# yavuzmurattas/Infrared-Colorization-with-ResNet-Generator-and-PatchGAN

Hardware: AMD Instinct MI355X
Metric: GAN train-step img/s (G+D fwd/bwd) at 256×256, 1/2/4/8 MI355X (higher is better)
Workload: dtype bf16; 1 GPU; GAN train step 256x256, batch 16/GPU, bf16 (BASELINE configs[1]); global_batch=16, img_size=256, height=256, width=256, parallelism=dp1

## Files before the change

### include/irgan.h

```cpp
#ifndef IRGAN_H
#define IRGAN_H
#include <stdint.h>
#include <stddef.h>

#if defined(__GNUC__) || defined(__clang__)
#define IRGAN_API __attribute__((visibility("default")))
#else
#define IRGAN_API
#endif

#ifdef __cplusplus
extern "C" {
#endif

typedef void* irgan_stream_t;

IRGAN_API int irgan_build_id(char* buf, int32_t len);

enum { IRGAN_F32 = 0, IRGAN_BF16 = 1, IRGAN_FP8 = 2 };
enum { IRGAN_PAD_ZERO = 0, IRGAN_PAD_REFLECT = 1 };
enum { IRGAN_ACT_NONE = 0, IRGAN_ACT_RELU = 1, IRGAN_ACT_LRELU = 2, IRGAN_ACT_TANH = 3 };
enum { IRGAN_OK = 0, IRGAN_EINVAL = 1001, IRGAN_EUNSUPPORTED = 1002 };

typedef struct irgan_conv_desc {
    int32_t N, H, W, Cin, ldx, xoff;
    int32_t Ho, Wo, Cout, ldy, yoff;
    int32_t OH, OW, omy, ooy, omx, oox;
    int32_t KH, KW, sy, sx, c0y, c0x;
    int32_t pad_mode;
    int32_t act;
    int32_t accumulate;
    int32_t dtype;
    int32_t out_dtype;
    int32_t mask_act;
    int32_t ldm, moff;
    int32_t cin_real;
    int32_t flags;
} irgan_conv_desc;
enum { IRGAN_CONV_DETERMINISTIC = 1 };

IRGAN_API int irgan_conv_fwd(const irgan_conv_desc* d, const void* x, const void* w,
                   const float* bias, void* y, const void* mask, irgan_stream_t s);

IRGAN_API int irgan_conv_fwd_stats(const irgan_conv_desc* d, const void* x, const void* w,
                         const float* bias, void* y, void* part, int32_t* nb, irgan_stream_t s);

IRGAN_API int irgan_conv_fwd_fp8(const irgan_conv_desc* d, const void* x, const void* w, const float* dqx,
                       const float* dqw, const float* bias, void* y, void* part, int32_t* nb,
                       irgan_stream_t s);

IRGAN_API int irgan_conv_wgrad_fp8(const irgan_conv_desc* d, const void* x8, const void* dy8, const float* dqx,
                         const float* dqdy, float* dw, float* ws, int64_t ws_floats, irgan_stream_t s);

enum { IRGAN_FP8_AMAX_PARTS = 256 };

IRGAN_API int irgan_fp8_quant(const void* x, int32_t dt, int64_t P, int32_t C, int32_t ldx, int32_t xoff,
                    void* y, int32_t ldy, int32_t yoff, const float* q, uint32_t* amax,
                    irgan_stream_t s);
IRGAN_API int irgan_fp8_scale(uint32_t* amax, int32_t n, float* q, float* dq, int32_t reset, irgan_stream_t s);
typedef struct irgan_fp8_job {
    const void* src;
    void* dst;
    int64_t n;
    int32_t slot, reserved;
} irgan_fp8_job;
IRGAN_API int irgan_fp8_quant_batch(const void* jobs, int32_t njobs, int64_t max_n, const float* q,
                          uint32_t* amax, irgan_stream_t s);

// ... 276 lines not shown
```

### infrared-colorization-with-resnet-generator-and-patchgan_amd/csrc/conv_pp.hip

```cpp
#include "conv_pp_kernel.h"

namespace irgan_res64 {
bool ok(const irgan_conv_desc* d);
int launch(const irgan_conv_desc* d, const void* x, const void* w, const float* bias, void* y, const void* mask,
           float2* part, hipStream_t st, void* ypool = nullptr);
}

namespace {

constexpr bool use_one(int) { return true; }
constexpr bool split128(int) { return true; }

#ifndef PP_BN_MODEL
#define PP_BN_MODEL 1
#endif
int narrow_bn(const irgan_conv_desc* d) {
    const long patches = (long)d->N * irgan_cdiv(d->Ho, PH) * irgan_cdiv(d->Wo, PW);
    if (patches * (d->Cout / 256) >= 160) {
        if (PP_BN_MODEL) {
            const long cus = irgan_cu_count();
            const long r256 = irgan_cdiv(patches * (d->Cout / 256), cus);
            const long r128 = irgan_cdiv(patches * (d->Cout / 128), cus);
            if (r128 * 0.575 <= 0.9 * r256) return 128;
        }
// ... 196 lines not shown
#define PPS(KHV, BNV, ONEV, ...)                                                                                   \
    conv_pp_kernel<KHV, KHV, BNV, false, true, false, ONEV, ##__VA_ARGS__><<<blocks, 512, 0, st>>>(                  \
        *d, (const bf16_t*)x, (const bf16_t*)w, bias, y, nullptr, ntn, tpx, tpy, swz, (float2*)part)
    const bool one = bn == 64 && use_one(d->Cin);
    if (s2d) {
        if (bn == 256) PPS(2, 256, false, true);
        else if (bn == 128) PPS(2, 128, false, true);
        else PPS(2, 64, true, true);
    } else if (k33) {
        if (bn == 256) PPS(3, 256, false);
        else if (bn == 128) PPS(3, 128, false);
        else { if (one) PPS(3, 64, true); else PPS(3, 64, false); }
    } else {
        if (bn == 256) PPS(4, 256, false);
        else if (bn == 128) PPS(4, 128, false);
        else { if (one) PPS(4, 64, true); else PPS(4, 64, false); }
    }
#undef PPS
    IRGAN_LAUNCH_CHECK();
    *nb = tpx * tpy;
    return 0;
}

extern "C" int irgan_conv_fwd_pool(const irgan_conv_desc* d, const void* x, const void* w, const float* bias, void* y,
                                   void* yp, irgan_stream_t s) {
    if (!d || !x || !w || !yp) return IRGAN_EINVAL;
    if ((long)d->N * d->Ho * d->Wo <= 0) return 0;
    if (!irgan_res64::ok(d) || d->accumulate || d->mask_act || d->Ho % 2 || d->Wo % 2 || d->Ho != d->OH ||
        d->Wo != d->OW || d->omy != 1 || d->omx != 1 || d->ooy || d->oox ||
        (long)d->N * (d->Ho / 2) * (d->Wo / 2) * d->Cout * 2 >= (1L << 31))
        return IRGAN_EUNSUPPORTED;
    irgan_res64::launch(d, x, w, bias, y, nullptr, nullptr, (hipStream_t)s, yp);
    IRGAN_LAUNCH_CHECK();
    return 0;
}

extern "C" int irgan_conv_fwd_fp8(const irgan_conv_desc* d, const void* x, const void* w, const float* dqx,
                                  const float* dqw, const float* bias, void* y, void* part, int32_t* nb,
                                  irgan_stream_t s) {
    if (!d || !x || !w || !dqx || !dqw || !y || (part && !nb)) return IRGAN_EINVAL;
    if ((long)d->N * d->Ho * d->Wo <= 0 || d->Cout <= 0) return 0;
    const bool k33 = d->KH == 3 && d->KW == 3;
    if (d->dtype != IRGAN_FP8 || d->out_dtype != IRGAN_BF16 || d->act == IRGAN_ACT_TANH || d->sy != 1 || d->sx != 1 ||
        d->Cin % 128 || !k33 || d->Cout % 64 || d->Cout == 192 || d->ldx % 16 || d->xoff % 16 || d->mask_act ||
        (long)d->N * d->H * d->W * d->ldx >= (1L << 30) || (long)d->Cout * 9 * d->Cin >= (1L << 30))
        return IRGAN_EUNSUPPORTED;
// ... 26 lines not shown
```

### infrared-colorization-with-resnet-generator-and-patchgan_amd/csrc/conv_pp_kernel.h

```cpp

#pragma once
#include <type_traits>

#include "conv_epilogue.h"

#ifndef PP_EXP
#define PP_EXP 0
#endif
#define PPX(b) ((PP_EXP & (b)) != 0)

namespace {

IRGAN_HD int lds_off(int row, int chunk) { return row * 128 + ((chunk ^ (row & 7)) << 4); }

IRGAN_HD void sched_fence() { __builtin_amdgcn_sched_barrier(0); }
IRGAN_HD void phase_barrier() {
    sched_fence();
#if !PPX(8)
    lds_barrier();
#endif
    sched_fence();
}
IRGAN_HD void wait_lgkm0() { asm volatile("s_waitcnt lgkmcnt(0)" ::: "memory"); }

constexpr int PH = 16, PW = 16;
constexpr int HPMAX = 46;
constexpr int HBYTES = HPMAX * 1024;
// ... 29 lines not shown
    };
    if (row) {
        const int line = y == 1 ? 0 : 1;
        add(line, x + 1);
        if (x == 1) { add(line, 0); add(2, y + 1); }
        if (x == W - 2) { add(line, W + 1); add(3, y + 1); }
    } else {
        add(x == 1 ? 2 : 3, y + 1);
    }
}
IRGAN_HD void ring_line_apply(const float (&v)[8], uint4& o) {
    const uint32_t wd[4] = {o.x, o.y, o.z, o.w};
    uint32_t o4[4];
#pragma unroll
    for (int k = 0; k < 4; ++k)
        o4[k] = pk_bf16(__uint_as_float(wd[k] << 16) + v[2 * k], __uint_as_float(wd[k] & 0xffff0000u) + v[2 * k + 1]);
    o = make_uint4(o4[0], o4[1], o4[2], o4[3]);
}

struct PhaseTab {
    const bf16_t* w[4];
    int c0y[4], c0x[4], ooy[4], oox[4];
};
IRGAN_HD int pick4(const int (&a)[4], int i) { return i == 0 ? a[0] : (i == 1 ? a[1] : (i == 2 ? a[2] : a[3])); }

template <int KH, int KW, int BN, bool ACC, bool STATS = false, bool F8 = false, bool ONE = false, bool S2D = false,
          bool PH4 = false>
__global__ __launch_bounds__(512, ONE ? 2 : 1) void conv_pp_kernel(const irgan_conv_desc d, const bf16_t* __restrict__ x,
                                                         const bf16_t* __restrict__ w, const float* __restrict__ bias,
                                                         void* __restrict__ y, const void* __restrict__ mask,
                                                         int ntn, int tpx, int tpy, int swz,
                                                         float2* __restrict__ part = nullptr,
                                                         const float* __restrict__ dqx = nullptr,
                                                         const float* __restrict__ dqw = nullptr,
                                                         const float* __restrict__ rg = nullptr,
                                                         const PhaseTab tab = PhaseTab{}) {
    constexpr int ESZ = F8 ? 1 : 2, CHN = 128 / ESZ;
    const char* const xb = (const char*)x;
    const char* wb = (const char*)w;
    constexpr int TAPS = KH * KW, HWd = PW + KW - 1, HROWS = (PH + KH - 1) * HWd, HP = (HROWS + 7) / 8;
    constexpr int BBYTES = PP<BN>::BBYTES, NJ = PP<BN>::NJ, WU = PP<BN>::WU, RSB = PP<BN>::RSB;
    constexpr int LDS = ONE ? HBYTES + 2 * BBYTES : PP<BN>::LDS;
    static_assert(!ONE || (BN == 64 && 256 * RSB <= LDS && !F8), "single-halo variant: staging must fit");
    constexpr int MI = PP<BN>::MIW, RW = PP<BN>::RW;
    constexpr int HS = 2;
    constexpr int NP = F8 ? MI / 2 : 1, NQ = F8 ? NJ / 2 : 1;
    static_assert(!F8 || (MI % 2 == 0 && NJ % 2 == 0), "fp8: 32 x 32 fragments");
    static_assert(HP <= HPMAX && HP > 32 && TAPS >= 2, "halo pieces per wave are 4 to 6");
    static_assert(!S2D || (KH == 2 && KW == 2 && !F8), "space-to-depth: the 2x2 form of a 4x4 stride-2 conv");
    static_assert(!PH4 || (!S2D && !F8 && !STATS), "four-phase backward-data: plain bf16");
    __shared__ __attribute__((aligned(1024))) char smem[LDS];
    char* const sH = smem;
    char* const sB = smem + (ONE ? 1 : 2) * HBYTES;

    const int tid = threadIdx.x, lane = tid & 63;
    const int wid = __builtin_amdgcn_readfirstlane(tid >> 6);
    const int grp = wid >> 2, wn = wid & 3;
    const int prow = grp * 8 + (wn % RW) * MI;
    const int cb = (wn / RW) * NJ * 16;
    int t = xcd_tile(blockIdx.x, gridDim.x, swz);
    const int nt = t % ntn;
    t /= ntn;
    int c0y = d.c0y, c0x = d.c0x, ooy = d.ooy, oox = d.oox;
    if constexpr (PH4) {
        const int ph = t & 3;
        t >>= 2;
        c0y = pick4(tab.c0y, ph);
        c0x = pick4(tab.c0x, ph);
        ooy = pick4(tab.ooy, ph);
        oox = pick4(tab.oox, ph);
        wb = (const char*)(ph == 0 ? tab.w[0] : (ph == 1 ? tab.w[1] : (ph == 2 ? tab.w[2] : tab.w[3])));
    }
    const int pxi = t % tpx;
    t /= tpx;
// ... 28 lines not shown
    const uint32_t wbytes = (uint32_t)((long)d.Cout * Kw * ESZ);
    const uint32_t b_off = (uint32_t)((n0 + wid * WU * 8 + sub) * Kw * ESZ + chunk * 16);
    auto issue_halo = [&](int c) {
        char* dst = sH + (ONE ? 0 : (c & 1) * HBYTES);
        const int cc = S2D ? c % cpp : c, ph = S2D ? c / cpp : 0;
        const i32x4 rs = make_rsrc(xb + cc * 128, xbytes - cc * 128);
        int lsub = sub;
        asm volatile("" : "+v"(lsub));
#pragma unroll
        for (int u = 0; u < 6; ++u)
            if (u < nh) blds16(rs, halo_off(u, lsub, ph), dst + (u * 8 + wid) * 1024);
    };
    auto issue_w = [&](int c, int tp, int stage) {
        int kcol = tp * d.Cin + c * CHN;
        if constexpr (S2D) {
            const int ph = c / cpp;
            kcol = ((2 * (tp >> 1) + (ph >> 1)) * 4 + 2 * (tp & 1) + (ph & 1)) * d.Cin + (c % cpp) * CHN;
        }
        const i32x4 rs = make_rsrc(wb + kcol * ESZ, wbytes - kcol * ESZ);
        char* dst = sB + stage * BBYTES + wid * WU * 1024;
#pragma unroll
        for (int u = 0; u < WU; ++u) blds16(rs, b_off, (uint32_t)(u * 8 * Kw * ESZ), dst + u * 1024);
    };
    auto reload_halo = [&](int c) {
        issue_halo(c);
        wait_vmcnt<0>();
        phase_barrier();
    };
    auto retire = [&](bool halo_now) {
        if (!halo_now) wait_vmcnt<0>();
        else if (nh == 6) wait_vmcnt<6>();
        else if (nh == 5) wait_vmcnt<5>();
        else wait_vmcnt<4>();
    };

    f32x4 acc[F8 ? 1 : MI][F8 ? 1 : NJ];
    f32x16 acc32[NP][NQ];
    if constexpr (F8) {
#pragma unroll
        for (int p = 0; p < NP; ++p)
#pragma unroll
            for (int q = 0; q < NQ; ++q)
#pragma unroll
                for (int r = 0; r < 16; ++r) acc32[p][q][r] = 0.f;
    } else {
#pragma unroll
        for (int i = 0; i < MI; ++i)
#pragma unroll
            for (int j = 0; j < NJ; ++j) acc[i][j] = f32x4{0.f, 0.f, 0.f, 0.f};
    }
    uint4 af[F8 ? 1 : MI], bfr[F8 ? 1 : NJ];
    v8i_t pf8[NP], wf8[NQ];
    issue_w(0, 0, 0);
    issue_halo(0);
    issue_w(0, 1, 1);
    wait_vmcnt<WU>();
    phase_barrier();
    if (grp == 1) phase_barrier();

    const int arow0 = (prow + (F8 ? (lane >> 4) & 1 : 0)) * HWd + (lane & 15);
    const int brow0 = cb + (lane & (F8 ? 31 : 15));
    const int g0 = F8 ? lane >> 5 : lane >> 4;
    const int bb0 = lds_off(brow0, g0), bb1 = lds_off(brow0, 4 + g0);
    int tsw[8];
#pragma unroll
    for (int k8 = 0; k8 < 8; ++k8) tsw[k8] = (g0 ^ ((arow0 + k8) & 7)) << 4;
#pragma unroll 1
    for (int c = 0; c < nchunk; ++c) {
        const int hb = arow0 * 128 + (ONE ? 0 : (c & 1) * HBYTES);
        const bool more = c + 1 < nchunk;
#pragma unroll
        for (int tp = 0; tp < TAPS; ++tp) {
            const int ty = tp / KW, tx = tp % KW;
            const int k = c * TAPS + tp;
            const char* B = sB + (k & 1) * BBYTES;
            const bool last_k = !more && tp == TAPS - 1;
            const bool halo_now = tp == 0 && more && !ONE;
            const bool reload = ONE && more && tp == TAPS - 1;
#pragma unroll
            for (int h = 0; h < HS; ++h) {
                const int bb = h ? bb1 : bb0;
                int hbp = hb;
                asm volatile("" : "+v"(hbp));
                if constexpr (F8) {
#pragma unroll
                    for (int q = 0; q < NQ; ++q)
                        wf8[q] = cat8(*(const i32x4*)(B + bb + q * 4096), *(const i32x4*)(B + (bb ^ 32) + q * 4096));
#pragma unroll
                    for (int p = 0; p < NP; ++p) {
                        const int K = (2 * p + ty) * HWd + tx;
                        const int sw = tsw[K & 7] ^ (h * 64);
                        pf8[p] = cat8(*(const i32x4*)(sH + (hbp + sw) + K * 128),
                                      *(const i32x4*)(sH + (hbp + (sw ^ 32)) + K * 128));
                    }
                } else {
#if !PPX(4)
#pragma unroll
                for (int j = 0; j < NJ; ++j) bfr[j] = *(const uint4*)(B + bb + j * 2048);
#pragma unroll
                for (int i = 0; i < MI; ++i) {
                    const int K = (i + ty) * HWd + tx;
                    af[i] = *(const uint4*)(sH + (hbp + (tsw[K & 7] ^ (h * 64))) + K * 128);
                }
#else
                if (k == 0 && h == 0) {
#pragma unroll
// ... 336 lines not shown
```

### infrared-colorization-with-resnet-generator-and-patchgan_amd/csrc/norm_rows.h

```cpp
#pragma once
#include "common.h"

#include <algorithm>
#include <initializer_list>

namespace {

constexpr int TPB = 256;
constexpr int V = 8;
constexpr int FC = 8, FS = 32;

struct Slice {
    const void* p;
    int dt, ld, off;
};
struct OSlice {
    void* p;
    int dt, ld, off;
};


inline bool dt_ok(int dt) { return dt == IRGAN_F32 || dt == IRGAN_BF16; }
inline bool act_ok(int act) { return act >= IRGAN_ACT_NONE && act <= IRGAN_ACT_LRELU; }
inline bool slice_ok(int C, int ld, int off) { return off >= 0 && (long)off + C <= ld; }
// ... 60 lines not shown
            u.z = pk_bf16(v[4], v[5]);
            u.w = pk_bf16(v[6], v[7]);
            *(uint4*)((bf16_t*)p + i) = u;
        } else {
            *(float4*)((float*)p + i) = make_float4(v[0], v[1], v[2], v[3]);
            *(float4*)((float*)p + i + 4) = make_float4(v[4], v[5], v[6], v[7]);
        }
    } else {
        stv(p, dt, i, v[0]);
    }
}

IRGAN_HD float act_fwd(float h, int act) {
    if (act == IRGAN_ACT_RELU) return h > 0.f ? h : 0.f;
    if (act == IRGAN_ACT_LRELU) return h > 0.f ? h : 0.2f * h;
    return h;
}
IRGAN_HD float act_grad(float h, int act) {
    if (act == IRGAN_ACT_RELU) return h > 0.f ? 1.f : 0.f;
    if (act == IRGAN_ACT_LRELU) return h > 0.f ? 1.f : 0.2f;
    return 1.f;
}

struct Lay {
    int CL, RP, cl, rl;
    __device__ Lay(int C, int VW) {
        CL = (C + VW - 1) / VW;
        if (CL > TPB) CL = TPB;
        RP = TPB / CL;
        cl = threadIdx.x % CL;
        rl = threadIdx.x / CL;
    }
    __device__ Lay(int CL_, int RP_, int cl_, int rl_) : CL(CL_), RP(RP_), cl(cl_), rl(rl_) {}
};

enum RowOrder { ROWS_TREE, ROWS_CHAINS };
IRGAN_HD bool rows_tree_ok(int CL) { return CL <= 64 && (64 % CL) == 0; }
IRGAN_HD RowOrder in_row_order(int CL) { return rows_tree_ok(CL) ? ROWS_TREE : ROWS_CHAINS; }

template <typename T, int VW, typename Emit>
IRGAN_HD void block_reduce(T* a0, T* a1, const Lay& L, RowOrder order, bool on, int cb, int c, int C, T* s0, T* s1,
                           Emit emit) {
    if (order == ROWS_TREE) {
        for (int o = L.CL; o < 64; o <<= 1) {
#pragma unroll
            for (int k = 0; k < VW; ++k) {
// ... 67 lines not shown
```

### infrared-colorization-with-resnet-generator-and-patchgan_amd/engine.py

```python
from __future__ import annotations

import math
import os
from collections import OrderedDict
from contextlib import nullcontext as _nullcontext
from typing import NamedTuple

import torch

from . import ops
from .ops import (ACT_LRELU, ACT_NONE, ACT_RELU, ACT_TANH, BF16, F32, PAD_REFLECT, PAD_ZERO, ConvSpec, Feat,
                  PackedConv)

IMAGENET_MEAN = (0.485, 0.456, 0.406)
IMAGENET_STD = (0.229, 0.224, 0.225)



def g_param_shapes(input_nc=1, output_nc=3, ngf=64, n_blocks=9, no_antialias=False, no_antialias_up=False,
                   use_bias=True, padding_type="reflect", use_dropout=False, batch_norm=False):
    s = OrderedDict()
    use_bias = use_bias and not batch_norm

    def conv(key, shape, normed=True):
# ... 287 lines not shown
    @staticmethod
    def _red(bufs: Buffers, N, C):
        return bufs.flat("in_red", 2 * N * C)

    @staticmethod
    def _no_fp8():
        raise NotImplementedError("the fp8 path runs with InstanceNorm (norm='instance')")

    def fwd(self, bufs: Buffers, name: str, x: Feat, y: Feat, act, res: Feat = None, xhat=None, nb=0, q8=None):
        mr = self._stats(bufs, name, x, nb)
        ops.in_apply(x, mr, y, act=act, res=res, xhat=xhat, q8=q8 and q8.side)
        if q8 is not None:
            q8.finish(y)

    def _stats(self, bufs: Buffers, name: str, x: Feat, nb):
        work = self._work(bufs, x.N, x.C)
        mr = bufs.get("mr_" + name, (x.N * x.C * 2,), torch.float32)
        if nb:
            ops.in_finalize(x, work, nb, mr)
        else:
            ops.in_stats(x, work, mr)
        return mr

    def _conv(self, bufs: Buffers, pc, x: Feat, z: Feat, conv8=None):
        work = self._work(bufs, z.N, z.C)
        if conv8 is not None:
            w8, dqw, x8, dqx = conv8
            return ops.conv_fwd_fp8(pc, w8, dqw, x8, dqx, z, part=work)
        nb = ops.conv_fwd_stats(pc, x, z, work) if INLayer.fused_stats else 0
        if not nb:
            ops.conv_fwd(pc, x, z)
        return nb

    def conv_fwd(self, bufs: Buffers, name: str, pc, x: Feat, z: Feat, y: Feat, act, res: Feat = None, conv8=None,
                 q8=None):
        self.fwd(bufs, name, z, y, act, res=res, nb=self._conv(bufs, pc, x, z, conv8), q8=q8)

    def conv_stats(self, bufs: Buffers, name: str, pc, x: Feat, z: Feat, conv8=None):
        return self._stats(bufs, name, z, self._conv(bufs, pc, x, z, conv8))

    def resample_fwd(self, bufs: Buffers, name: str, pc, x: Feat, z: Feat, a_name: str, act, y: Feat, fused, plain,
                     conv8=None, q8=None):
        mr = self.conv_stats(bufs, name, pc, x, z, conv8=conv8)
        side = q8.side if q8 is not None else None
        taken = INLayer.fused_resample and (fused(z, mr, act, y, q8=side) if side is not None else
                                            fused(z, mr, act, y))
        if not taken:
            a = Feat(bufs.get(a_name, (z.N, z.H, z.W, z.C), z.t.dtype))
            ops.in_apply(z, mr, a, act=act)
            plain(a, y)
        if q8 is not None:
            q8.finish(y, taken)

    def bwd(self, bufs: Buffers, name: str, dy: Feat, z: Feat, act, dx: Feat, db=None, dy2: Feat = None, q8=None,
            wgrad=True):
        N, C = z.N, z.C
        work = self._work(bufs, N, C)
        red = self._red(bufs, N, C)
        mr = bufs.d["mr_" + name]
        ops.in_backward(dy, z, act, mr, work, red, dx, db=db if INLayer.sum_bias_grad else None, dy2=dy2,
                        q8=q8.side if q8 is not None and not INLayer.sum_bias_grad else None)
        if q8 is not None:
# ... 221 lines not shown
        A = self.eng.f8a
        if st.calib and self.s_calib is not None:
            return st.x1_8c, A.dqp(self.s_calib)
        return st.x8[self.name], ops.Pi(st.dq_used, self.rec.s_x) if used else A.dqp(self.rec.s_x)

    def _conv8(self, st):
        return (*self._w8(self.rec.w_fwd), *self._x8(st)) if st.on[self.group] else None

    def feed(self, st, x: Feat):
        if st.on[self.group]:
            self.eng.f8a.quant(self.rec.s_x, x, st.x8[self.name], record=not st.frozen)

    def side(self, st, sl=None):
        if not st.on[self.group] or (st.calib and self.group == "ud"):
            return None
        x8 = st.x8[self.name]
        return ops.Fp8Out(self.eng.f8a, self.rec.s_x, x8.sl(*sl) if sl else x8, record=not st.frozen)

    def calibrate(self, st, x: Feat):
        if st.calib and self.group == "ud":
            slot, x8 = (self.s_calib, st.x1_8c) if self.s_calib is not None else (self.rec.s_x, st.x8[self.name])
            self.eng.f8a.calibrate(slot, x, x8)

    def fwd(self, g: Buffers, st, x: Feat, z: Feat, y: Feat, act, res: Feat = None, nxt: "GenConv" = None):
        if self.xp:
            xp = Feat(g.get(self.xp, (x.N, x.H + 2, x.W + 2, x.C), self.eng.tdt))
            ops.pad(x, xp, 1, "replicate")
            x = xp
        self.norm.conv_fwd(g, self.name, self.pc, x, z, y, act, res=res, conv8=self._conv8(st),
                           q8=nxt.side(st) if nxt else None)

    def resample_fwd(self, g: Buffers, st, x: Feat, z: Feat, a_name, act, y: Feat, fused, plain):
        self.norm.resample_fwd(g, self.name, self.pc, x, z, a_name, act, y, fused, plain, conv8=self._conv8(st))

    def bwd(self, g: Buffers, st, dy: Feat, z: Feat, act, dz: Feat, x: Feat, dx: Feat, accumulate=False, padbuf=None,
            pend: list = None, resample=None):
        e, on = self.eng, st.on[self.group]
        dz8 = Feat(g.get(self.dy8, (*dz.t.shape[:3], dz.C), torch.float8_e4m3fn)) if on else None
        db, q8 = e._bgrad(self.key + ".bias"), ops.Fp8Out(e.f8a, self.rec.s_dy, dz8) if on else None
        if resample is not None:
            self.norm.resample_bwd(g, self.name, dy, z, act, dz, *resample, db=db, q8=q8)
        else:
            self.norm.bwd(g, self.name, dy, z, act, dz, db=db, q8=q8)
        if on:
            self._wgrad(st, x, dz, dz8)
            if self.s_calib is not None:
                st.x1_8c = None
            ops.conv_dgrad_fp8(self.pc, *self._w8(self.rec.w_flip), dz8, e.f8a.dqp(self.rec.s_dy), dz, dx,
                               accumulate=accumulate)
            return
        if self.group != "res":
            self._wgrad(st, x, dz)
        if self.xp:
# ... 188 lines not shown
        self.norms["inc"].conv_fwd(g, "inc", self.inc, ir_t, z0, x0, ACT_RELU)
        if self.no_aa:
            z1 = Feat(g.get("z1", (B, H1, W1, c1), T))
            ops.conv_fwd(self.down1, x0, z1)
            self.norms["down1"].fwd(g, "down1", z1, x1, ACT_RELU)
        else:
            z1 = Feat(g.get("z1", (B, H, W, c1), T))
            self.norms["down1"].resample_fwd(g, "down1", self.down1, x0, z1, "a1", ACT_RELU, x1, ops.blur_down_in,
                                             ops.blur_down, q8=D2.side(st))
            D2.calibrate(st, x1)
        h = Feat(g.get("h0", (B, H2, W2, c2), T))
        if self.no_aa:
            z2 = Feat(g.get("z2", (B, H2, W2, c2), T))
            ops.conv_fwd(self.down2, x1, z2)
            self.norms["down2"].fwd(g, "down2", z2, h, ACT_RELU)
        else:
            z2 = Feat(g.get("z2", (B, H1, W1, c2), T))
            D2.resample_fwd(g, st, x1, z2, "a2", ACT_RELU, h, ops.blur_down_in, ops.blur_down)
        if self.blocks:
            self.blocks[0][0].feed(st, h)
        for b, (ra, rb) in enumerate(self.blocks):
            r1 = Feat(g.get(f"r1_{b}", (B, H2, W2, c2), T))
            t = None if t8_only else Feat(g.get(f"t{b}", (B, H2, W2, c2), T))
            ra.fwd(g, st, h, r1, t, ACT_RELU, nxt=rb)
            if self.use_dropout and train:
                t, t1 = Feat(g.get(f"td{b}", (B, H2, W2, c2), T)), t
                ops.dropout(t1, t, g.state["dropout_seed"] + 2 * b)
            r2 = Feat(g.get(f"r2_{b}", (B, H2, W2, c2), T))
            hn = Feat(g.get(f"h{b + 1}", (B, H2, W2, c2), T))
            rb.fwd(g, st, t, r2, hn, ACT_NONE, res=h, nxt=self.blocks[b + 1][0] if b + 1 < self.n_blocks else None)
            h = hn
        self._fp8_roll(st, "res", "fwd", snapshot=True)
        y1 = Feat(cat1, 0, c2)
        if self.no_aa_up:
            self._convt(self.up1_up, h, y1, g, "ut1")
        else:
            q8 = U1.side(st, (0, c2))
            ops.upsample(h, y1, q8=q8 and q8.side)
        U1.calibrate(st, Feat(cat1))
        z3 = Feat(g.get("z3", (B, H1, W1, c1), T))
        y2 = Feat(cat2, 0, c1)
        if self.no_aa_up:
            a3 = Feat(g.get("a3", (B, H1, W1, c1), T))
            U1.fwd(g, st, Feat(cat1), z3, a3, ACT_RELU)
            self._convt(self.up2_up, a3, y2, g, "ut2")
        else:
            U1.resample_fwd(g, st, Feat(cat1), z3, "a3", ACT_RELU, y2, ops.upsample_in, ops.upsample)
        self._fp8_roll(st, "ud", "cat", snapshot=True)
        z4 = Feat(g.get("z4", (B, H, W, c0), T))
        a4 = Feat(g.get("a4", (B, H, W, c0), T))
        self.norms["up2"].conv_fwd(g, "up2", self.up2, Feat(cat2), z4, a4, ACT_RELU)
        fake = g.get("fake", (B, H, W, self.output_nc), torch.float32)
        ops.conv_fwd(self.outc, a4, Feat(fake), act=ACT_TANH)
# ... 132 lines not shown
        self.packs = [_pc(store, k, ConvSpec(chans[i], chans[i + 1], 4, s, 1, PAD_ZERO), dtype)
                      for i, (k, s, _) in enumerate(self.LAYERS)]
        self.norms = [make_norm(norm, store, f"model.{int(k.split('.')[1]) + 1}") if n else None
                      for (k, _, n) in self.LAYERS]
        self.norm_type, self.training = norm, True
        self.bn_sync = None
        self.bufs = Buffers(store.device)

    def pack(self):
        if self._pack_batch is None:
            self._pack_batch = ops.PackBatch(self.packs)
        self._pack_batch.run()

    def forward(self, din: Feat, tag="", bufs: Buffers = None, groups: int = 1, bn_sync: bool = False) -> torch.Tensor:
        g, T = bufs or self.bufs, self.tdt
        if self.norm_type == "batch":
            for nrm in self.norms:
                if nrm is not None:
                    nrm.configure(training=self.training, groups=groups, repeat=1,
                                  sync=self.bn_sync if bn_sync else None)
        x = din
        acts, pre = [din], {}
        g.state[tag] = (acts, pre)
        for i, pc in enumerate(self.packs):
            Ho, Wo = pc.spec.out_hw(x.H, x.W)
            last = i == len(self.packs) - 1
            y = Feat(g.get(f"{tag}e{i}", (x.N, Ho, Wo, pc.spec.cout), torch.float32 if last else T))
            if i == 0:
                ops.conv_fwd(pc, x, y, act=ACT_LRELU)
            elif last:
                if not ops.patch_head_fwd(pc, x, y.t):
                    ops.conv_fwd(pc, x, y)
            else:
                z = Feat(g.get(f"{tag}z{i}", (x.N, Ho, Wo, pc.spec.cout), T))
                self.norms[i].conv_fwd(g, f"{tag}n{i}", pc, x, z, y, ACT_LRELU)
                pre[i] = z
            acts.append(y)
            x = y
        return x.t

    def backward(self, dout: torch.Tensor, want_wgrad=True, want_dinput=False, tag="", bufs: Buffers = None,
                 ready=None):
        g, T, S = bufs or self.bufs, self.tdt, self.store
        acts, pre = g.state[tag]
        G = S.grad
        n = len(self.packs)
        def logits_grad():
            dbuf = g.zeros(f"{tag}dout_t", tuple(dout.shape[:3]) + (8,), T)
            ops.axpby(Feat(dout), 1.0, Feat(dbuf, 0, dout.shape[3]))
            return Feat(dbuf, 0, self.packs[-1].cout_eff)
        dy = None
        for i in reversed(range(n)):
            pc, key = self.packs[i], self.LAYERS[i][0]
            x = acts[i]
            if dy is None and not (i == n - 1 and ops.is_patch_head(pc, x)):
                dy = logits_grad()
            bias_sum = None
            if i == n - 1:
# ... 438 lines not shown
```

### infrared-colorization-with-resnet-generator-and-patchgan_amd/ops.py

```python
from __future__ import annotations

import ctypes
import math
import os

import torch

from . import _lib
from ._lib import (ACT_LRELU, ACT_NONE, ACT_RELU, ACT_TANH, BF16, F32, FP8, IN_PARTS, PAD_REFLECT,
                   PAD_ZERO)

TORCH_DT = {F32: torch.float32, BF16: torch.bfloat16, FP8: torch.float8_e4m3fn}


def dt_code(t: torch.Tensor) -> int:
    if t.dtype == torch.float32:
        return F32
    if t.dtype == torch.bfloat16:
        return BF16
    if t.dtype == torch.float8_e4m3fn:
        return FP8
    raise TypeError(f"unsupported dtype {t.dtype}")


# ... 289 lines not shown
    Ho, Wo = s.out_hw(x.H, x.W)
    if pc.dtype != BF16 or yp.dt != BF16 or yp.off or yp.ld != s.cout or Ho % 2 or Wo % 2:
        return False
    assert (yp.N, yp.H, yp.W, yp.C) == (x.N, Ho // 2, Wo // 2, s.cout) and x.C == pc.cin_eff
    if y is not None:
        assert (y.H, y.W, y.C, y.N, y.dt) == (Ho, Wo, s.cout, x.N, BF16)
    d = _fwd_desc(s, x, y if y is not None else yp, pc.cin_eff, pc.dtype, BF16, act, y_sized=y is not None)
    return TIMER.wrap(conv_tag("fwdpool", s, (x.H, x.W), x.N), lambda: _try(
        "irgan_conv_fwd_pool", ctypes.byref(d), x.ptr, P(pc.fwd), P(pc.bias), y.ptr if y is not None else None,
        yp.ptr, stream()))


def conv_fwd_stats(pc: PackedConv, x: Feat, y: Feat, part: torch.Tensor) -> int:
    s = pc.spec
    if pc.dtype != BF16 or y.dt != BF16 or s.cout % 64 or s.cout == 192 or (s.stride != 1 and s.k != 4):
        return 0
    assert y.C == s.cout and x.C == pc.cin_eff, "conv_fwd shape mismatch"
    d = _fwd_desc(s, x, y, pc.cin_eff, pc.dtype, y.dt, cin_real=s.cin if s.cin < pc.cin_eff else 0)
    nb = ctypes.c_int32(0)
    ran = TIMER.wrap(conv_tag("fwd", s, (x.H, x.W), x.N), lambda: _try(
        "irgan_conv_fwd_stats", ctypes.byref(d), x.ptr, P(pc.fwd), P(pc.bias), y.ptr, P(part), ctypes.byref(nb),
        stream()))
    return int(nb.value) if ran else 0


PATCH_HEAD = [os.environ.get("IRGAN_NO_PATCH_HEAD") != "1"]


def is_patch_head(pc: PackedConv, x: Feat) -> bool:
    s = pc.spec
    return (PATCH_HEAD[0] and pc.dtype == BF16 and x.dt == BF16 and s.cout == 1 and s.k == 4 and s.stride == 1
            and s.pad == 1 and s.mode == PAD_ZERO and s.cin == x.C == 512)


def patch_head_fwd(pc: PackedConv, x: Feat, y: torch.Tensor) -> bool:
    if not is_patch_head(pc, x):
        return False
    assert y.dtype == torch.float32 and tuple(y.shape) == (x.N, x.H - 1, x.W - 1, 1) and y.is_contiguous()

    ws = _wgrad_ws(y.device)

    return TIMER.wrap(conv_tag("fwd", pc.spec, (x.H, x.W), x.N), lambda: _try(
        "irgan_patch_head_fwd", x.ptr, x.N, x.H, x.W, x.C, x.ld, x.off, P(pc.fwd),
        P(pc.bias) if pc.bias is not None else None, P(y), P(ws), ws.numel(), stream()))


# ... 893 lines not shown
```

Before: 1323 img/s.

## Fuse instance-norm apply and activation into next conv's halo load

```diff
diff --git a/include/irgan.h b/include/irgan.h
--- a/include/irgan.h
+++ b/include/irgan.h
@@ -44,6 +44,14 @@
 
 IRGAN_API int irgan_conv_fwd_stats(const irgan_conv_desc* d, const void* x, const void* w,
                          const float* bias, void* y, void* part, int32_t* nb, irgan_stream_t s);
+
+IRGAN_API int irgan_conv_fwd_norm_in(const irgan_conv_desc* d, const void* z_in, const float* mr, int32_t act_in,
+                           const void* res, const void* xhat, const void* t8, void* t_out, int32_t ldt,
+                           int32_t toff, const void* w, const float* bias, void* y, irgan_stream_t s);
+IRGAN_API int irgan_conv_fwd_norm_in_stats(const irgan_conv_desc* d, const void* z_in, const float* mr,
+                                 int32_t act_in, const void* res, const void* xhat, const void* t8, void* t_out,
+                                 int32_t ldt, int32_t toff, const void* w, const float* bias, void* y, void* part,
+                                 int32_t* nb, irgan_stream_t s);
 
 IRGAN_API int irgan_conv_fwd_fp8(const irgan_conv_desc* d, const void* x, const void* w, const float* dqx,
                        const float* dqw, const float* bias, void* y, void* part, int32_t* nb,
diff --git a/infrared-colorization-with-resnet-generator-and-patchgan_amd/csrc/conv_pp.hip b/infrared-colorization-with-resnet-generator-and-patchgan_amd/csrc/conv_pp.hip
--- a/infrared-colorization-with-resnet-generator-and-patchgan_amd/csrc/conv_pp.hip
+++ b/infrared-colorization-with-resnet-generator-and-patchgan_amd/csrc/conv_pp.hip
@@ -242,6 +242,77 @@
     return 0;
 }
 
+namespace {
+
+template <int KH, int BN, bool STATS, bool S2D>
+void launch_norm_in(const irgan_conv_desc* d, const void* z, const void* w, const float* bias, void* y, void* part,
+                    const NormIn& ni, hipStream_t st) {
+    const int tpx = irgan_cdiv(d->Wo, PW), tpy = irgan_cdiv(d->Ho, PH), ntn = d->Cout / BN;
+    conv_pp_kernel<KH, KH, BN, false, STATS, false, false, S2D, false, true><<<d->N * tpy * tpx * ntn, 512, 0, st>>>(
+        *d, (const bf16_t*)z, (const bf16_t*)w, bias, y, nullptr, ntn, tpx, tpy, irgan_xcd_swz(), (float2*)part, nullptr,
+        nullptr, nullptr, PhaseTab{}, ni);
+}
+
+template <bool STATS>
+int norm_in_run(const irgan_conv_desc* d, const void* z_in, const float* mr, int act_in, const void* res,
+                const void* xhat, const void* t8, void* t_out, int ldt, int toff, const void* w, const float* bias,
+                void* y, void* part, int32_t* nb, hipStream_t st) {
+    if (!d || !z_in || !mr || !t_out || !w || !y || (STATS && (!part || !nb))) return IRGAN_EINVAL;
+    static const bool use_pp = !getenv("IRGAN_NO_PP");
+    const bool k33 = d->KH == 3 && d->KW == 3, k44 = d->KH == 4 && d->KW == 4;
+    const bool s2d = k44 && d->sy == 2 && d->sx == 2;
+    if (!use_pp || res || xhat || t8 || act_in < IRGAN_ACT_NONE || act_in > IRGAN_ACT_LRELU)
+        return IRGAN_EUNSUPPORTED;
+    if (d->dtype != IRGAN_BF16 || d->out_dtype != IRGAN_BF16 || d->accumulate || d->mask_act ||
+        d->act == IRGAN_ACT_TANH || ((d->sy != 1 || d->sx != 1) && !s2d) || !(k33 || k44) || d->Cin % 64 ||
+        d->Cin > 512 || d->Cout % 64 || d->ldx % 8 || d->xoff % 8 || ldt % 8 || toff % 8 || toff < 0 ||
+        toff + d->Cin > ldt || (long)d->N * d->H * d->W * d->ldx >= (1L << 30) ||
+        (long)d->Cout * d->KH * d->KW * d->Cin >= (1L << 30) || (long)d->N * d->Ho * d->Wo <= 0 || irgan_res64::ok(d))
+        return IRGAN_EUNSUPPORTED;
+    if (STATS && (d->act != IRGAN_ACT_NONE || d->Cout == 192 || d->ldy % 8 || d->yoff % 8 || d->Ho != d->OH ||
+                  d->Wo != d->OW || d->omy != 1 || d->omx != 1 || d->ooy || d->oox))
+        return IRGAN_EUNSUPPORTED;
+    const int tpx = irgan_cdiv(d->Wo, PW), tpy = irgan_cdiv(d->Ho, PH);
+    if (STATS && tpx * tpy > IRGAN_IN_PARTS) return IRGAN_EUNSUPPORTED;
+    const int kh = s2d ? 2 : d->KH;
+    if (d->c0y > 0 || d->c0x > 0 || d->c0y <= -d->KH || d->c0x <= -d->KW) return IRGAN_EUNSUPPORTED;
+    const int ey = (tpy - 1) * PH + PH + kh - 2, ex = (tpx - 1) * PW + PW + kh - 2;
+    if ((s2d ? 2 * ey + 1 + d->c0y : ey + d->c0y) < d->H - 1 || (s2d ? 2 * ex + 1 + d->c0x : ex + d->c0x) < d->W - 1)
+        return IRGAN_EUNSUPPORTED;
+    const int bn = d->Cout % 256 == 0 ? narrow_bn(d) : 64;
+    if (bn == 64) return IRGAN_EUNSUPPORTED;
+    const NormIn ni{mr, (bf16_t*)t_out, act_in, ldt, toff};
+#define PNI(KHV, S2DV)                                                                        \
+    do {                                                                                      \
+        if (bn == 256) launch_norm_in<KHV, 256, STATS, S2DV>(d, z_in, w, bias, y, part, ni, st); \
+        else launch_norm_in<KHV, 128, STATS, S2DV>(d, z_in, w, bias, y, part, ni, st);           \
+    } while (0)
+    if (s2d) PNI(2, true);
+    else if (k33) PNI(3, false);
+    else PNI(4, false);
+#undef PNI
+    IRGAN_LAUNCH_CHECK();
+    if (STATS) *nb = tpx * tpy;
+    return 0;
+}
+
+}
+
+extern "C" int irgan_conv_fwd_norm_in(const irgan_conv_desc* d, const void* z_in, const float* mr, int32_t act_in,
+                                      const void* res, const void* xhat, const void* t8, void* t_out, int32_t ldt,
+                                      int32_t toff, const void* w, const float* bias, void* y, irgan_stream_t s) {
+    return norm_in_run<false>(d, z_in, mr, act_in, res, xhat, t8, t_out, ldt, toff, w, bias, y, nullptr, nullptr,
+                              (hipStream_t)s);
+}
+
+extern "C" int irgan_conv_fwd_norm_in_stats(const irgan_conv_desc* d, const void* z_in, const float* mr, int32_t act_in,
+                                            const void* res, const void* xhat, const void* t8, void* t_out, int32_t ldt,
+                                            int32_t toff, const void* w, const float* bias, void* y, void* part,
+                                            int32_t* nb, irgan_stream_t s) {
+    return norm_in_run<true>(d, z_in, mr, act_in, res, xhat, t8, t_out, ldt, toff, w, bias, y, part, nb,
+                             (hipStream_t)s);
+}
+
 extern "C" int irgan_conv_fwd_pool(const irgan_conv_desc* d, const void* x, const void* w, const float* bias, void* y,
                                    void* yp, irgan_stream_t s) {
     if (!d || !x || !w || !yp) return IRGAN_EINVAL;
diff --git a/infrared-colorization-with-resnet-generator-and-patchgan_amd/csrc/conv_pp_kernel.h b/infrared-colorization-with-resnet-generator-and-patchgan_amd/csrc/conv_pp_kernel.h
--- a/infrared-colorization-with-resnet-generator-and-patchgan_amd/csrc/conv_pp_kernel.h
+++ b/infrared-colorization-with-resnet-generator-and-patchgan_amd/csrc/conv_pp_kernel.h
@@ -3,6 +3,7 @@
 #include <type_traits>
 
 #include "conv_epilogue.h"
+#include "norm_rows.h"
 
 #ifndef PP_EXP
 #define PP_EXP 0
@@ -78,10 +79,16 @@
     const bf16_t* w[4];
     int c0y[4], c0x[4], ooy[4], oox[4];
 };
+struct NormIn {
+    const float* mr;
+    bf16_t* t;
+    int act, ldt, toff;
+};
+
 IRGAN_HD int pick4(const int (&a)[4], int i) { return i == 0 ? a[0] : (i == 1 ? a[1] : (i == 2 ? a[2] : a[3])); }
 
 template <int KH, int KW, int BN, bool ACC, bool STATS = false, bool F8 = false, bool ONE = false, bool S2D = false,
-          bool PH4 = false>
+          bool PH4 = false, bool NORM_IN = false>
 __global__ __launch_bounds__(512, ONE ? 2 : 1) void conv_pp_kernel(const irgan_conv_desc d, const bf16_t* __restrict__ x,
                                                          const bf16_t* __restrict__ w, const float* __restrict__ bias,
                                                          void* __restrict__ y, const void* __restrict__ mask,
@@ -90,7 +97,8 @@
                                                          const float* __restrict__ dqx = nullptr,
                                                          const float* __restrict__ dqw = nullptr,
                                                          const float* __restrict__ rg = nullptr,
-                                                         const PhaseTab tab = PhaseTab{}) {
+                                                         const PhaseTab tab = PhaseTab{},
+                                                         const NormIn ni = NormIn{}) {
     constexpr int ESZ = F8 ? 1 : 2, CHN = 128 / ESZ;
     const char* const xb = (const char*)x;
     const char* wb = (const char*)w;
@@ -105,7 +113,9 @@
     static_assert(HP <= HPMAX && HP > 32 && TAPS >= 2, "halo pieces per wave are 4 to 6");
     static_assert(!S2D || (KH == 2 && KW == 2 && !F8), "space-to-depth: the 2x2 form of a 4x4 stride-2 conv");
     static_assert(!PH4 || (!S2D && !F8 && !STATS), "four-phase backward-data: plain bf16");
-    __shared__ __attribute__((aligned(1024))) char smem[LDS];
+    static_assert(!NORM_IN || (!F8 && !PH4 && !ACC && !ONE), "normalise-on-load: plain bf16 forward, two halo buffers");
+    constexpr int NTBL = NORM_IN ? 4096 : 0;
+    __shared__ __attribute__((aligned(1024))) char smem[LDS + NTBL];
     char* const sH = smem;
     char* const sB = smem + (ONE ? 1 : 2) * HBYTES;
 
@@ -180,6 +190,57 @@
 #pragma unroll
         for (int u = 0; u < WU; ++u) blds16(rs, b_off, (uint32_t)(u * 8 * Kw * ESZ), dst + u * 1024);
     };
+    auto piece_px = [&](int u, int lsub, int ph, int& iy, int& ix, bool& live, bool& mine) {
+        const int h = (u * 8 + wid) * 8 + lsub;
+        const int hy = h / HWd, hx = h - hy * HWd;
+        iy = py0 + hy + c0y;
+        ix = px0 + hx + c0x;
+        if constexpr (S2D) {
+            iy = 2 * (py0 + hy) + (ph >> 1) + c0y;
+            ix = 2 * (px0 + hx) + (ph & 1) + c0x;
+        }
+        const int ry = reflect ? reflect_idx(iy, d.H) : iy, rx = reflect ? reflect_idx(ix, d.W) : ix;
+        live = (h < HROWS) & ((unsigned)ry < (unsigned)d.H) & ((unsigned)rx < (unsigned)d.W);
+        const int loy = S2D ? 0 : -c0y, lox = S2D ? 0 : -c0x;
+        mine = (nt == 0) & (h < HROWS) & ((unsigned)iy < (unsigned)d.H) & ((unsigned)ix < (unsigned)d.W) &
+               (hy >= loy) & ((hy < loy + PH) | (pyi == tpy - 1)) & (hx >= lox) & ((hx < lox + PW) | (pxi == tpx - 1));
+    };
+    auto t_ptr = [&](int cc, int lsub, int iy, int ix) {
+        return (uint4*)(ni.t + ((long)(img * d.H + iy) * d.W + ix) * ni.ldt + ni.toff + cc * 64 +
+                        ((lane & 7) ^ lsub) * 8);
+    };
+    auto norm_piece = [&](int u, int c, bool store) {
+        const int cc = S2D ? c % cpp : c, ph = S2D ? c / cpp : 0;
+        int iy, ix, lsub = sub;
+        asm volatile("" : "+v"(lsub));
+        bool live, mine;
+        piece_px(u, lsub, ph, iy, ix, live, mine);
+        uint4* p = (uint4*)(sH + (c & 1) * HBYTES + (u * 8 + wid) * 1024 + lsub * 128 + (lane & 7) * 16);
+        const float4* m4 = (const float4*)(smem + LDS) + cc * 32 + ((lane & 7) ^ lsub) * 4;
+        float mean[8], rstd[8];
+#pragma unroll
+        for (int k = 0; k < 4; ++k) {
+            const float4 e = m4[k];
+            mean[2 * k] = e.x; rstd[2 * k] = e.y; mean[2 * k + 1] = e.z; rstd[2 * k + 1] = e.w;
+        }
+        const uint4 raw = *p;
+        uint4 o = in_apply_pk8(raw, mean, rstd, ni.act);
+        if (!live) o = raw;
+        *p = o;
+        if (store && mine) *t_ptr(cc, lsub, iy, ix) = o;
+    };
+    auto store_piece = [&](int u) {
+        int iy, ix, lsub = sub;
+        asm volatile("" : "+v"(lsub));
+        bool live, mine;
+        piece_px(u, lsub, 0, iy, ix, live, mine);
+        if (mine) *t_ptr(0, lsub, iy, ix) = *(const uint4*)(sH + (u * 8 + wid) * 1024 + lsub * 128 + (lane & 7) * 16);
+    };
+    auto norm_chunk = [&](int c, bool store) {
+#pragma unroll
+        for (int u = 0; u < 6; ++u)
+            if (u < nh) norm_piece(u, c, store);
+    };
     auto reload_halo = [&](int c) {
         issue_halo(c);
         wait_vmcnt<0>();
@@ -209,11 +270,26 @@
     }
     uint4 af[F8 ? 1 : MI], bfr[F8 ? 1 : NJ];
     v8i_t pf8[NP], wf8[NQ];
+    float tv[2];
+    if constexpr (NORM_IN) {
+#pragma unroll
+        for (int i = 0; i < 2; ++i) tv[i] = tid + 512 * i < 2 * d.Cin ? ni.mr[(long)img * d.Cin * 2 + tid + 512 * i] : 0.f;
+    }
     issue_w(0, 0, 0);
     issue_halo(0);
+    if constexpr (NORM_IN) {
+#pragma unroll
+        for (int i = 0; i < 2; ++i) ((float*)(smem + LDS))[tid + 512 * i] = tv[i];
+    }
     issue_w(0, 1, 1);
     wait_vmcnt<WU>();
+    if constexpr (NORM_IN) wait_lgkm0();
     phase_barrier();
+    if constexpr (NORM_IN) {
+        norm_chunk(0, nchunk == 1);
+        wait_lgkm0();
+        phase_barrier();
+    }
     if (grp == 1) phase_barrier();
 
     const int arow0 = (prow + (F8 ? (lane >> 4) & 1 : 0)) * HWd + (lane & 15);
@@ -240,6 +316,20 @@
                 const int bb = h ? bb1 : bb0;
                 int hbp = hb;
                 asm volatile("" : "+v"(hbp));
+                if constexpr (NORM_IN) {
+                    constexpr int PPP = (6 + (TAPS - 2) * HS - 1) / ((TAPS - 2) * HS);
+                    if (more && tp >= 2) {
+#pragma unroll
+                        for (int u = ((tp - 2) * HS + h) * PPP; u < ((tp - 2) * HS + h + 1) * PPP && u < 6; ++u)
+                            if (u < nh) norm_piece(u, c + 1, true);
+                    }
+                    if (tp == 1 && h == 0 && c == 0 && more) {
+#pragma unroll
+                        for (int u = 0; u < 6; ++u)
+                            if (u < nh) store_piece(u);
+                    }
+                    sched_fence();
+                }
                 if constexpr (F8) {
 #pragma unroll
                     for (int q = 0; q < NQ; ++q)
diff --git a/infrared-colorization-with-resnet-generator-and-patchgan_amd/csrc/norm_rows.h b/infrared-colorization-with-resnet-generator-and-patchgan_amd/csrc/norm_rows.h
--- a/infrared-colorization-with-resnet-generator-and-patchgan_amd/csrc/norm_rows.h
+++ b/infrared-colorization-with-resnet-generator-and-patchgan_amd/csrc/norm_rows.h
@@ -106,6 +106,24 @@
     return 1.f;
 }
 
+IRGAN_HD uint4 in_apply_pk8(const uint4 x, const float* mean, const float* rstd, int act) {
+    float xv[8], o[8];
+    bf8f(x, xv);
+    const bool relu = act == IRGAN_ACT_RELU, lrelu = act == IRGAN_ACT_LRELU;
+#pragma unroll
+    for (int k = 0; k < 8; ++k) {
+        const float h = (xv[k] - mean[k]) * rstd[k];
+        const float neg = relu ? 0.f : (lrelu ? 0.2f * h : h);
+        o[k] = h > 0.f ? h : neg;
+    }
+    uint4 w;
+    w.x = pk_bf16(o[0], o[1]);
+    w.y = pk_bf16(o[2], o[3]);
+    w.z = pk_bf16(o[4], o[5]);
+    w.w = pk_bf16(o[6], o[7]);
+    return w;
+}
+
 struct Lay {
     int CL, RP, cl, rl;
     __device__ Lay(int C, int VW) {
diff --git a/infrared-colorization-with-resnet-generator-and-patchgan_amd/engine.py b/infrared-colorization-with-resnet-generator-and-patchgan_amd/engine.py
--- a/infrared-colorization-with-resnet-generator-and-patchgan_amd/engine.py
+++ b/infrared-colorization-with-resnet-generator-and-patchgan_amd/engine.py
@@ -333,22 +333,37 @@
             ops.in_stats(x, work, mr)
         return mr
 
-    def _conv(self, bufs: Buffers, pc, x: Feat, z: Feat, conv8=None):
+    @staticmethod
+    def takes_pre(*norms) -> bool:
+        return all(type(n) is INLayer for n in norms)
+
+    def _conv(self, bufs: Buffers, pc, x: Feat, z: Feat, conv8=None, pre=None):
         work = self._work(bufs, z.N, z.C)
         if conv8 is not None:
             w8, dqw, x8, dqx = conv8
             return ops.conv_fwd_fp8(pc, w8, dqw, x8, dqx, z, part=work)
+        if pre is not None:
+            z_in, mr, act = pre
+            if not INLayer.fused_stats:
+                ops.conv_fwd_norm_in(pc, z_in, mr, act, x, z)
+                return 0
+            nb = ops.conv_fwd_norm_in_stats(pc, z_in, mr, act, x, z, work)
+            if not nb:
+                ops.conv_fwd(pc, x, z)
+            return nb
         nb = ops.conv_fwd_stats(pc, x, z, work) if INLayer.fused_stats else 0
         if not nb:
             ops.conv_fwd(pc, x, z)
         return nb
 
     def conv_fwd(self, bufs: Buffers, name: str, pc, x: Feat, z: Feat, y: Feat, act, res: Feat = None, conv8=None,
-                 q8=None):
-        self.fwd(bufs, name, z, y, act, res=res, nb=self._conv(bufs, pc, x, z, conv8), q8=q8)
-
-    def conv_stats(self, bufs: Buffers, name: str, pc, x: Feat, z: Feat, conv8=None):
-        return self._stats(bufs, name, z, self._conv(bufs, pc, x, z, conv8))
+                 q8=None, pre=None):
+        nb = self._conv(bufs, pc, x, z, conv8, pre=pre) if pre is not None else self._conv(bufs, pc, x, z, conv8)
+        self.fwd(bufs, name, z, y, act, res=res, nb=nb, q8=q8)
+
+    def conv_stats(self, bufs: Buffers, name: str, pc, x: Feat, z: Feat, conv8=None, pre=None):
+        nb = self._conv(bufs, pc, x, z, conv8, pre=pre) if pre is not None else self._conv(bufs, pc, x, z, conv8)
+        return self._stats(bufs, name, z, nb)
 
     def resample_fwd(self, bufs: Buffers, name: str, pc, x: Feat, z: Feat, a_name: str, act, y: Feat, fused, plain,
                      conv8=None, q8=None):
@@ -616,13 +631,28 @@
             slot, x8 = (self.s_calib, st.x1_8c) if self.s_calib is not None else (self.rec.s_x, st.x8[self.name])
             self.eng.f8a.calibrate(slot, x, x8)
 
-    def fwd(self, g: Buffers, st, x: Feat, z: Feat, y: Feat, act, res: Feat = None, nxt: "GenConv" = None):
+    def fwd(self, g: Buffers, st, x: Feat, z: Feat, y: Feat, act, res: Feat = None, nxt: "GenConv" = None,
+            pre=None):
         if self.xp:
             xp = Feat(g.get(self.xp, (x.N, x.H + 2, x.W + 2, x.C), self.eng.tdt))
             ops.pad(x, xp, 1, "replicate")
             x = xp
+        if pre is not None:
+            self.norm.conv_fwd(g, self.name, self.pc, x, z, y, act, res=res, pre=pre)
+            return
         self.norm.conv_fwd(g, self.name, self.pc, x, z, y, act, res=res, conv8=self._conv8(st),
                            q8=nxt.side(st) if nxt else None)
+
+    def hands_apply_to(self, st, nxt: "GenConv") -> bool:
+        return (ops.CONV_NORM_IN[0] and INLayer.takes_pre(self.norm, nxt.norm) and not nxt.xp
+                and not st.on[self.group] and not st.on[nxt.group])
+
+    def stats_fwd(self, g: Buffers, st, x: Feat, z: Feat):
+        if self.xp:
+            xp = Feat(g.get(self.xp, (x.N, x.H + 2, x.W + 2, x.C), self.eng.tdt))
+            ops.pad(x, xp, 1, "replicate")
+            x = xp
+        return self.norm.conv_stats(g, self.name, self.pc, x, z)
 
     def resample_fwd(self, g: Buffers, st, x: Feat, z: Feat, a_name, act, y: Feat, fused, plain):
         self.norm.resample_fwd(g, self.name, self.pc, x, z, a_name, act, y, fused, plain, conv8=self._conv8(st))
@@ -857,13 +887,18 @@
         for b, (ra, rb) in enumerate(self.blocks):
             r1 = Feat(g.get(f"r1_{b}", (B, H2, W2, c2), T))
             t = None if t8_only else Feat(g.get(f"t{b}", (B, H2, W2, c2), T))
-            ra.fwd(g, st, h, r1, t, ACT_RELU, nxt=rb)
+            pre = None
+            if t is not None and not (self.use_dropout and train) and ra.hands_apply_to(st, rb):
+                pre = (r1, ra.stats_fwd(g, st, h, r1), ACT_RELU)
+            else:
+                ra.fwd(g, st, h, r1, t, ACT_RELU, nxt=rb)
             if self.use_dropout and train:
                 t, t1 = Feat(g.get(f"td{b}", (B, H2, W2, c2), T)), t
                 ops.dropout(t1, t, g.state["dropout_seed"] + 2 * b)
             r2 = Feat(g.get(f"r2_{b}", (B, H2, W2, c2), T))
             hn = Feat(g.get(f"h{b + 1}", (B, H2, W2, c2), T))
-            rb.fwd(g, st, t, r2, hn, ACT_NONE, res=h, nxt=self.blocks[b + 1][0] if b + 1 < self.n_blocks else None)
+            rb.fwd(g, st, t, r2, hn, ACT_NONE, res=h, nxt=self.blocks[b + 1][0] if b + 1 < self.n_blocks else None,
+                   pre=pre)
             h = hn
         self._fp8_roll(st, "res", "fwd", snapshot=True)
         y1 = Feat(cat1, 0, c2)
@@ -1042,6 +1077,7 @@
         x = din
         acts, pre = [din], {}
         g.state[tag] = (acts, pre)
+        pend = None
         for i, pc in enumerate(self.packs):
             Ho, Wo = pc.spec.out_hw(x.H, x.W)
             last = i == len(self.packs) - 1
@@ -1053,7 +1089,14 @@
                     ops.conv_fwd(pc, x, y)
             else:
                 z = Feat(g.get(f"{tag}z{i}", (x.N, Ho, Wo, pc.spec.cout), T))
-                self.norms[i].conv_fwd(g, f"{tag}n{i}", pc, x, z, y, ACT_LRELU)
+                kw = {"pre": pend} if pend is not None else {}
+                hand = (ops.CONV_NORM_IN[0] and self.dtype == BF16 and i + 2 < len(self.packs)
+                        and INLayer.takes_pre(self.norms[i], self.norms[i + 1]))
+                if hand:
+                    pend = (z, self.norms[i].conv_stats(g, f"{tag}n{i}", pc, x, z, **kw), ACT_LRELU)
+                else:
+                    self.norms[i].conv_fwd(g, f"{tag}n{i}", pc, x, z, y, ACT_LRELU, **kw)
+                    pend = None
                 pre[i] = z
             acts.append(y)
             x = y
diff --git a/infrared-colorization-with-resnet-generator-and-patchgan_amd/ops.py b/infrared-colorization-with-resnet-generator-and-patchgan_amd/ops.py
--- a/infrared-colorization-with-resnet-generator-and-patchgan_amd/ops.py
+++ b/infrared-colorization-with-resnet-generator-and-patchgan_amd/ops.py
@@ -335,6 +335,48 @@
         "irgan_conv_fwd_stats", ctypes.byref(d), x.ptr, P(pc.fwd), P(pc.bias), y.ptr, P(part), ctypes.byref(nb),
         stream()))
     return int(nb.value) if ran else 0
+
+
+CONV_NORM_IN = [os.environ.get("IRGAN_CONV_NORM_IN") != "0"]
+
+
+def set_conv_norm_in(on: bool) -> bool:
+    old, CONV_NORM_IN[0] = CONV_NORM_IN[0], bool(on)
+    return old
+
+
+def _norm_in_args(pc: PackedConv, z_in: Feat, mr, act_in, t: Feat, y: Feat, res, xhat, q8, act=ACT_NONE):
+    s = pc.spec
+    if not CONV_NORM_IN[0] or z_in.dt != pc.dtype or t.dt != pc.dtype:
+        return None
+    assert y.C == s.cout and z_in.C == t.C == pc.cin_eff and (t.N, t.H, t.W) == (z_in.N, z_in.H, z_in.W), \
+        "conv_fwd_norm_in shape mismatch"
+    assert not _shares_bytes(z_in, t), "conv_fwd_norm_in: t must not overlap z_in"
+    d = _fwd_desc(s, z_in, y, pc.cin_eff, pc.dtype, y.dt, act, cin_real=s.cin if s.cin < pc.cin_eff else 0)
+    return (ctypes.byref(d), z_in.ptr, P(mr), act_in, res.ptr if res else None, P(xhat),
+            q8[0].ptr if q8 is not None else None, t.ptr, t.ld, t.off, P(pc.fwd), P(pc.bias)), d
+
+
+def conv_fwd_norm_in(pc: PackedConv, z_in: Feat, mr, act_in, t: Feat, y: Feat, act=ACT_NONE, res: Feat = None,
+                     xhat: torch.Tensor = None, q8=None):
+    a = _norm_in_args(pc, z_in, mr, act_in, t, y, res, xhat, q8, act)
+    if a is not None and TIMER.wrap(conv_tag("fwd_nin", pc.spec, (z_in.H, z_in.W), z_in.N), lambda: _try(
+            "irgan_conv_fwd_norm_in", *a[0], y.ptr, stream())):
+        return
+    in_apply(z_in, mr, t, act=act_in, res=res, xhat=xhat, q8=q8)
+    conv_fwd(pc, t, y, act=act)
+
+
+def conv_fwd_norm_in_stats(pc: PackedConv, z_in: Feat, mr, act_in, t: Feat, y: Feat, part: torch.Tensor,
+                           res: Feat = None, xhat: torch.Tensor = None, q8=None) -> int:
+    a = _norm_in_args(pc, z_in, mr, act_in, t, y, res, xhat, q8)
+    if a is not None:
+        nb = ctypes.c_int32(0)
+        if TIMER.wrap(conv_tag("fwd_nin", pc.spec, (z_in.H, z_in.W), z_in.N), lambda: _try(
+                "irgan_conv_fwd_norm_in_stats", *a[0], y.ptr, P(part), ctypes.byref(nb), stream())):
+            return int(nb.value)
+    in_apply(z_in, mr, t, act=act_in, res=res, xhat=xhat, q8=q8)
+    return conv_fwd_stats(pc, t, y, part)
 
 
 PATCH_HEAD = [os.environ.get("IRGAN_NO_PATCH_HEAD") != "1"]
```

Result: slower. 1309 img/s (-1.0%).
